# AegisIK/DistMLIP

Hardware: NVIDIA H100
Metric: atoms/sec (energy+forces) CHGNet a-Si r_cut=5A (higher is better)
Workload: dtype f32

## Files before the change

distmlip_b200/csrc/kernels.cu:

```cuda
#include "final_tail.cuh"
#include "kernels.cuh"
#include "wgmma.cuh"

#include <algorithm>

namespace b2m {

__device__ __forceinline__ float sigm(float x) {
  float e, r;
  asm("ex2.approx.ftz.f32 %0, %1;" : "=f"(e) : "f"(x * -1.4426950408889634f));
  asm("rcp.approx.ftz.f32 %0, %1;" : "=f"(r) : "f"(1.f + e));
  return r;
}
__device__ __forceinline__ float silu_f(float x) { return x * sigm(x); }
__device__ __forceinline__ float dsilu_f(float x) {
  float s = sigm(x);
  return s * (1.f + x * (1.f - s));
}

__device__ __forceinline__ uint32_t smem_u32(const void* p) { return (uint32_t)__cvta_generic_to_shared(p); }
__device__ __forceinline__ void mbar_init(uint64_t* bar, uint32_t count) {
  asm volatile("mbarrier.init.shared::cta.b64 [%0], %1;" ::"r"(smem_u32(bar)), "r"(count) : "memory");
}
__device__ __forceinline__ void fence_barrier_init() {
// ... 256 lines not shown
template <int ROWS>
__device__ __forceinline__ void issue_gather(const AtomConvArgs& a, int64_t t, const EdgeRow& row, int lr, float* buf,
                                             uint64_t* bar, int* s_src, int* s_dst, int* s_bond, float* s_d) {
  if (lr == 0) mbar_expect_tx(bar, (uint32_t)min((int64_t)ROWS, a.E - t * ROWS) * 512u);
  if (lr < ROWS) {
    if (s_src != nullptr) s_src[lr] = row.src;
    s_dst[lr] = row.dst;
    s_bond[lr] = row.bond;
    s_d[lr] = row.d;
    if (row.src >= 0) bulk_g2s(buf + lr * LDE, a.Aproj + (size_t)row.src * D2, 512u, bar);
  }
}
template <int ROWS>
__device__ __forceinline__ void radial_rows(const AtomConvArgs& a, const float* s_d, int nvalid, float* be_s, float* be8,
                                            float* dbe_s, float* dbe8) {
  const int r = threadIdx.x % ROWS, half = (threadIdx.x / ROWS) & 1;
  const float d = s_d[r];
  const int k0 = half ? 5 : 0, k1 = half ? 9 : 5;
  for (int k = k0; k < k1; k++) {
    float be = 0.f, dbe = 0.f;
    if (r < nvalid) rbf_env_k(d, a.rp.freq[k], a.rp, be, dbe);
    *(k < 8 ? be_s + r * 8 + k : be8 + r) = be;
    if (dbe_s != nullptr) *(k < 8 ? dbe_s + r * 8 + k : dbe8 + r) = dbe;
  }
}
__device__ __forceinline__ float2 ld_f2(const float* p) { return *reinterpret_cast<const float2*>(p); }
__device__ __forceinline__ void st_f2(float* p, float x, float y) { *reinterpret_cast<float2*>(p) = make_float2(x, y); }

__device__ __forceinline__ constexpr int fq(int ii, int j) { return 4 * (j >> 1) + 2 * ii + (j & 1); }

__device__ __forceinline__ void radial_mma(const Map& m, int h, const float* x_s, const float* img, float (&d)[32]) {
  const float2 u = ld_f2(x_s + m.row(2 * h) * 8 + m.cb), v = ld_f2(x_s + m.row(2 * h + 1) * 8 + m.cb);
  const float x[1][4] = {{u.x, v.x, u.y, v.y}};
  uint32_t b = s_u32(img);
  asm volatile("" : "+r"(b));
  wg_mma64(x, b, b + 512u * 4u, 0, false, d);
}

template <int R>
__device__ __forceinline__ void first_layer_half(const AtomConvArgs& a, const Map& m, int h, const float* tile,
                                                 const int* s_dst, const int* s_bond, const float* be_s,
                                                 const float* be8, const float* rad, int nvalid,
                                                 float (&acc)[R][AC]) {
  const int c0 = 64 * m.branch + m.cb;
  float2 cv[2][AC / 2], qv[2][AC / 2];
  float b8[2];
  bool viaQ[2], ok[2];
#pragma unroll
  for (int ii = 0; ii < 2; ii++) {
    const int r = m.row(2 * h + ii);
    const int dst = s_dst[r], bond = s_bond[r];
    ok[ii] = r < nvalid;
    viaQ[ii] = a.Qproj != nullptr && bond >= 0;
    const float* cp = a.Cproj + (size_t)max(dst, 0) * D2 + c0;
#pragma unroll
    for (int jj = 0; jj < AC / 2; jj++) cv[ii][jj] = dst >= 0 ? __ldg(reinterpret_cast<const float2*>(cp + 8 * jj)) : make_float2(0.f, 0.f);
    if (viaQ[ii]) {
      const float* qp = a.Qproj + (size_t)bond * D2 + c0;
#pragma unroll
      for (int jj = 0; jj < AC / 2; jj++) qv[ii][jj] = __ldg(reinterpret_cast<const float2*>(qp + 8 * jj));
    } else {
#pragma unroll
      for (int jj = 0; jj < AC / 2; jj++) qv[ii][jj] = make_float2(0.f, 0.f);
    }
    b8[ii] = be8[r];
  }
  float d[32];
  radial_mma(m, h, be_s, rad + ATOM_RAD_M + 1024 * m.branch, d);
#pragma unroll
  for (int j = 0; j < AC; j++) {
    const float m8 = rad[ATOM_RAD_M8 + 64 * m.branch + m.col(j)];
#pragma unroll
    for (int ii = 0; ii < 2; ii++) {
      const int r = m.row(2 * h + ii);
      const float x = tile[r * LDE + 64 * m.branch + m.col(j)];
      const float2 c2 = cv[ii][j >> 1], q2 = qv[ii][j >> 1];
      const float t = viaQ[ii] ? ((j & 1) ? q2.y : q2.x) : fmaf(b8[ii], m8, d[fq(ii, j)]);
      acc[2 * h + ii][j] = ok[ii] ? x + ((j & 1) ? c2.y : c2.x) + t : 0.f;
    }
  }
}

template <int R>
__device__ __forceinline__ void wg_mm64_acc(const float (&x)[R][AC], int h, const float* Bcan, float (&acc)[R][AC]) {
  float v[8][4];
#pragma unroll
  for (int ks = 0; ks < 8; ks++) {
    v[ks][0] = x[2 * h][2 * ks], v[ks][1] = x[2 * h + 1][2 * ks];
    v[ks][2] = x[2 * h][2 * ks + 1], v[ks][3] = x[2 * h + 1][2 * ks + 1];
  }
  const uint32_t b_hi = s_u32(Bcan);
  float d[32];
  wg_mma64(v, b_hi, b_hi + 4096u * 4u, 0, false, d);
#pragma unroll
  for (int q = 0; q < 32; q++) acc[2 * h + ((q >> 1) & 1)][2 * (q >> 2) + (q & 1)] = d[q];
}

__device__ __forceinline__ float quad_row_sum(const float (&v)[AR]) {
  const int l = threadIdx.x & 3;
  const bool b0 = l & 1, b1 = l & 2;
  float w[2];
#pragma unroll
  for (int h = 0; h < 2; h++)
    w[h] = (b0 ? v[2 * h + 1] : v[2 * h]) + __shfl_xor_sync(0xffffffffu, b0 ? v[2 * h] : v[2 * h + 1], 1);
  return (b1 ? w[1] : w[0]) + __shfl_xor_sync(0xffffffffu, b1 ? w[0] : w[1], 2);
}

__device__ __forceinline__ void red_add_v4(float* p, float4 v) {
  asm volatile("red.global.add.v4.f32 [%0], {%1, %2, %3, %4};" ::"l"(p), "f"(v.x), "f"(v.y), "f"(v.z), "f"(v.w)
               : "memory");
}

__device__ __forceinline__ void seg_add(float* out, int width, int col, int k, const float4& v, int& cur, float4& sum) {
  if (k != cur) {
    if (cur >= 0) red_add_v4(out + (size_t)cur * width + col, sum);
    cur = k;
    sum = make_float4(0.f, 0.f, 0.f, 0.f);
  }
  if (k >= 0) sum.x += v.x, sum.y += v.y, sum.z += v.z, sum.w += v.w;
}

template <int LPR, int ROWS = TM, int NTH = NT>
__device__ __forceinline__ void scatter_rows(const float* tile, const int* key0, float* out0, const int* key1,
                                             float* out1, const int* gidx, float* gat, const int* sidx = nullptr,
                                             float* sto = nullptr) {
  constexpr int R = ROWS * LPR / NTH, W = 4 * LPR, B = 8;
  static_assert(R % B == 0 && B % 4 == 0, "batches of B rows, their indices read as int4");
  const int t = threadIdx.x % NTH, q = t % LPR, r0 = t / LPR * R;
  float4 s0 = make_float4(0.f, 0.f, 0.f, 0.f), s1 = s0;
  int c0 = -1, c1 = -1;
#pragma unroll
  for (int b = 0; b < R; b += B) {
    float4 v[B];
    int k0[B], k1[B], kg[B], ks[B];
#pragma unroll
    for (int i = 0; i < B; i++) v[i] = *reinterpret_cast<const float4*>(tile + (r0 + b + i) * LDE + 4 * q);
    auto ld_idx = [&](const int* idx, bool on, int(&k)[B]) {
#pragma unroll
      for (int i = 0; i < B; i += 4) {
        const int4 x = on ? *reinterpret_cast<const int4*>(idx + r0 + b + i) : make_int4(-1, -1, -1, -1);
        k[i] = x.x, k[i + 1] = x.y, k[i + 2] = x.z, k[i + 3] = x.w;
      }
    };
    ld_idx(key0, out0 != nullptr, k0);
    ld_idx(key1, out1 != nullptr, k1);
    ld_idx(gidx, gat != nullptr, kg);
    ld_idx(sidx, sto != nullptr, ks);
#pragma unroll
    for (int i = 0; i < B; i++) {
      if (ks[i] >= 0) *reinterpret_cast<float4*>(sto + (size_t)ks[i] * W + 4 * q) = v[i];
      if (kg[i] >= 0) red_add_v4(gat + (size_t)kg[i] * W + 4 * q, v[i]);
      seg_add(out0, W, 4 * q, k0[i], v[i], c0, s0);
      seg_add(out1, W, 4 * q, k1[i], v[i], c1, s1);
    }
  }
  if (c0 >= 0) red_add_v4(out0 + (size_t)c0 * W + 4 * q, s0);
  if (c1 >= 0) red_add_v4(out1 + (size_t)c1 * W + 4 * q, s1);
}

constexpr int TW = 64;
constexpr int WGF = 3, NTF = 128 * WGF;
struct AtomSmemFwd {
  static constexpr int kTile = 32;
  static constexpr int kW = kTile + WGF * TW * LDE;
  static constexpr int kRad = kW + 16384;
  static constexpr int kBe = kRad + ATOM_RAD;
  static constexpr int kBe8 = kBe + WGF * TW * 8;
  static constexpr int kB2 = kBe8 + WGF * TW;
  static constexpr int kD = kB2 + 128;
  static constexpr int kIdx = kD + WGF * TW;
  static constexpr int kTotal = kIdx + 2 * WGF * TW;
  static constexpr size_t bytes = (size_t)kTotal * 4;
};
static_assert(AtomSmemFwd::bytes <= 232448, "atom-conv forward shared memory");
static_assert(AtomSmemFwd::kW % 4 == 0 && AtomSmemFwd::kRad % 4 == 0 && AtomSmemFwd::kBe % 4 == 0 &&
                  AtomSmemFwd::kIdx % 4 == 0,
              "16-byte aligned images, radial rows and index slots");

// ... 243 lines not shown
#pragma unroll
      for (int ii = 0; ii < 2; ii++)
#pragma unroll
        for (int jj = 0; jj < AC / 2; jj++) {
          float* p = P + m.row(ii) * LDE + c0 + m.col(2 * jj);
          const float2 pre = ld_f2(p);
          float& x0 = x[ii][2 * jj];
          float& x1 = x[ii][2 * jj + 1];
          x0 *= dsilu_f(pre.x);
          x1 *= dsilu_f(pre.y);
          st_f2(p, x0, x1);
        }
      float dm[32];
      radial_mma(m, 0, dbe_s, rad + ATOM_RAD_M + 1024 * mb.branch, dm);
#pragma unroll
      for (int ii = 0; ii < 2; ii++) {
        const int r = m.row(ii);
        const float db8 = dbe8[r];
        float s = 0.f;
#pragma unroll
        for (int jj = 0; jj < AC / 2; jj++) {
          const float2 mk = ld_f2(rad + ATOM_RAD_M8 + c0 + m.col(2 * jj));
          s = fmaf(x[ii][2 * jj], fmaf(db8, mk.x, dm[fq(ii, 2 * jj)]), s);
          s = fmaf(x[ii][2 * jj + 1], fmaf(db8, mk.y, dm[fq(ii, 2 * jj + 1)]), s);
        }
        if (r < nvalid && !(useQ && s_bond[r] >= 0)) sd[2 * mb.branch + ii] += s;
      }
    };
    reverse(mL, L);
    reverse(mG, G);
    {
      const float v = quad_row_sum(sd);
      const float v1 = __shfl_xor_sync(0xffffffffu, v, 2);
      const int r = m.row(tid & 1);
      if ((tid & 2) == 0 && r < nvalid) a.gd[e0 + r] += v + v1;
    }
    wg_sync(w);
    scatter_rows<32, TW, 128>(P, s_dst, a.gA != nullptr ? a.gC : nullptr, nullptr, nullptr, s_src, a.gA, s_bond,
                              useQ ? a.gQ : nullptr);
    fence_proxy_async_smem();
    wg_sync(w);
    if (t + step < ntiles) {
      issue_gather<TW>(a, t + step, nxt, lr, P, mbar, s_src, s_dst, s_bond, s_d);
      nxt = edge_row(a, (t + 2 * step) * TW + lr, lr < TW);
    }
  }
}

void launch_atomconv_bwd(cudaStream_t st, const AtomConvArgs& a, int num_sms) {
  if (a.E <= 0) return;
  static PerDeviceOnce attr;
  if (auto once_ = attr.first(); once_) {
    B2M_CK(cudaFuncSetAttribute(k_atomconv_bwd, cudaFuncAttributeMaxDynamicSharedMemorySize, (int)AtomSmemBwd::bytes));
  }
  launch(k_atomconv_bwd, std::min(cdiv(cdiv(a.E, TW), WGB), num_sms), NTB, AtomSmemBwd::bytes, st, a);
}

struct LineSmem {
  static constexpr int kBuf = 32;
  static constexpr int kW = kBuf + 2 * TM * LDE;
  static constexpr int kB2 = kW + 16384;
  static constexpr int kIdx = kB2 + 128;
  static constexpr int kTotal = kIdx + 6 * TM;
  static constexpr size_t bytes = (size_t)kTotal * 4;
};
static_assert(LineSmem::bytes <= 232448, "line-graph shared memory");

struct LineSm {
  float* smem;
  __device__ __forceinline__ uint64_t* hbar() const { return reinterpret_cast<uint64_t*>(smem); }
  __device__ __forceinline__ uint64_t* abar() const { return hbar() + 2; }
  __device__ __forceinline__ uint64_t* wbar() const { return hbar() + 4; }
  __device__ __forceinline__ float* buf(int s) const { return smem + LineSmem::kBuf + s * TM * LDE; }
  __device__ __forceinline__ float* W() const { return smem + LineSmem::kW; }
  __device__ __forceinline__ float* b2() const { return smem + LineSmem::kB2; }
  __device__ __forceinline__ int* idx(int s, int k) const {
    return reinterpret_cast<int*>(smem + LineSmem::kIdx) + (2 * k + s) * TM;
  }
};

struct AngleIdx {
  int a, b, c;
};
__device__ __forceinline__ AngleIdx angle_idx(const LineArgs& a, int64_t r) {
  AngleIdx x{-1, -1, -1};
  if (threadIdx.x < TM && r < a.A) {
    x.a = a.a_in[r];
    x.b = a.a_out[r];
    x.c = a.a_ctr[r];
  }
  return x;
}
__device__ __forceinline__ void line_issue_ha(const LineArgs& a, const LineSm& sm, int64_t t, const AngleIdx& x,
                                             float* buf, int s) {
  const int tid = threadIdx.x;
  if (tid == 0) mbar_expect_tx(&sm.hbar()[s], (uint32_t)min((int64_t)TM, a.A - t * TM) * 512u);
  if (tid < TM) {
    sm.idx(s, 0)[tid] = x.a;
    sm.idx(s, 1)[tid] = x.b;
    sm.idx(s, 2)[tid] = x.c;
    if (x.a >= 0) bulk_g2s(buf + tid * LDE, a.Ha + (size_t)x.a * D2, 512u, &sm.hbar()[s]);
  }
}
__device__ __forceinline__ void line_issue_ang(const LineArgs& a, const LineSm& sm, int64_t t, float* buf, int s) {
  const int tid = threadIdx.x;
  const int nvalid = (int)min((int64_t)TM, a.A - t * TM);
  if (tid == 0) mbar_expect_tx(&sm.abar()[s], (uint32_t)nvalid * 256u);
  if (tid < nvalid) bulk_g2s(buf + tid * LDE + 64, a.ang + (size_t)(t * TM + tid) * D, 256u, &sm.abar()[s]);
}
__device__ __forceinline__ AngleIdx line_prologue(const LineArgs& a, const LineSm& sm) {
  const int tid = threadIdx.x;
  if (tid == 0) {
    for (int i = 0; i < 5; i++) mbar_init(&sm.hbar()[i], 1);
    fence_barrier_init();
  }
  AngleIdx x = angle_idx(a, (int64_t)blockIdx.x * TM + tid);
  if (tid < 128) sm.b2()[tid] = a.b2 ? a.b2[tid] : 0.f;
  __syncthreads();
  if (tid == 0) bulk_g2s_image(sm.W(), a.Wgcan, 16384 * 4, sm.wbar());
  line_issue_ha(a, sm, blockIdx.x, x, sm.buf(0), 0);
  line_issue_ang(a, sm, blockIdx.x, sm.buf(1), 0);
  return angle_idx(a, ((int64_t)blockIdx.x + gridDim.x) * TM + tid);
}

__device__ __forceinline__ void line_first_layer(const LineArgs& a, const Map& m, const float* P, const int* s_b,
                                                 const int* s_c, int nvalid, float (&acc)[AR][AC]) {
  const int c0 = 64 * m.branch + m.cb;
#pragma unroll
  for (int i = 0; i < AR; i++) {
    const int r = m.row(i);
    const bool ok = r < nvalid;
    const float* hb = a.Hb + (size_t)(ok ? s_b[r] : 0) * D2 + c0;
    const float* xc = a.Xc + (size_t)(ok ? s_c[r] : 0) * D2 + c0;
    float2 hv[AC / 2], xv[AC / 2];
#pragma unroll
    for (int jj = 0; jj < AC / 2; jj++) {
      hv[jj] = ok ? __ldg(reinterpret_cast<const float2*>(hb + 8 * jj)) : make_float2(0.f, 0.f);
      xv[jj] = ok ? __ldg(reinterpret_cast<const float2*>(xc + 8 * jj)) : make_float2(0.f, 0.f);
    }
#pragma unroll
    for (int jj = 0; jj < AC / 2; jj++) {
      const float2 ha = ok ? ld_f2(P + r * LDE + c0 + 8 * jj) : make_float2(0.f, 0.f);
      float& x0 = acc[i][2 * jj];
      float& x1 = acc[i][2 * jj + 1];
      x0 = ok ? ha.x + x0 + hv[jj].x + xv[jj].x : 0.f;
      x1 = ok ? ha.y + x1 + hv[jj].y + xv[jj].y : 0.f;
    }
  }
}

__device__ __forceinline__ void red_add_v2(float* p, float x, float y) {
  asm volatile("red.global.add.v2.f32 [%0], {%1, %2};" ::"l"(p), "f"(x), "f"(y) : "memory");
}

template <bool HIDDEN>
__global__ void __launch_bounds__(NT, 1) k_line_fwd(const LineArgs a) {
  extern __shared__ __align__(128) float smem[];
  const LineSm sm{smem};
  const float* b2s = sm.b2();
  const int tid = threadIdx.x;
  const int64_t ntiles = (a.A + TM - 1) / TM, step = gridDim.x;
  AngleIdx nxt = line_prologue(a, sm);
  uint32_t wpar = 0;

  int it = 0;
  for (int64_t t = blockIdx.x; t < ntiles; t += step, it++) {
    const int s = it & 1;
    float* P = sm.buf(s);
    float* Q = sm.buf(s ^ 1);
    const int* s_b = sm.idx(s, 1);
    const int* s_c = sm.idx(s, 2);
    const int64_t r0 = t * TM;
    const int nvalid = (int)min((int64_t)TM, a.A - r0);
    const bool more = t + step < ntiles;
    const Map m;
    float acc[AR][AC];
    mbar_wait(&sm.abar()[s], stage_parity(it));
    mbar_wait(sm.wbar(), wpar);
    if (HIDDEN) wpar ^= 1;
    gemm64(Q, LDE, 64, sm.W() + m.branch * 8192, acc);
    fence_proxy_async_smem();
    __syncthreads();
    if (more) {
      line_issue_ha(a, sm, t + step, nxt, Q, s ^ 1);
      nxt = angle_idx(a, (t + 2 * step) * TM + tid);
    }
    if (HIDDEN && tid == 0) bulk_g2s_image(sm.W(), a.W2can, 16384 * 4, sm.wbar());
    mbar_wait(&sm.hbar()[s], stage_parity(it));
    line_first_layer(a, m, P, s_b, s_c, nvalid, acc);
#pragma unroll
    for (int i = 0; i < AR; i++)
#pragma unroll
      for (int j = 0; j < AC; j++) acc[i][j] = HIDDEN || m.branch == 0 ? silu_f(acc[i][j]) : sigm(acc[i][j]);
    if (HIDDEN) {
      mbar_wait(sm.wbar(), wpar);
      wpar ^= 1;
      wg_mm64_acc(acc, 0, sm.W() + m.branch * 8192, acc);
      wg_mm64_acc(acc, 1, sm.W() + m.branch * 8192, acc);
#pragma unroll
      for (int i = 0; i < AR; i++)
#pragma unroll
        for (int j = 0; j < AC; j++) {
          const float u = acc[i][j] + b2s[m.branch * 64 + m.col(j)];
          acc[i][j] = m.branch == 0 ? silu_f(u) : sigm(u);
        }
    }
    fence_proxy_async_smem();
    __syncthreads();
    if (more) {
      line_issue_ang(a, sm, t + step, P, s ^ 1);
      if (HIDDEN && tid == 0) bulk_g2s_image(sm.W(), a.Wgcan, 16384 * 4, sm.wbar());
    }
    if (m.branch == 1) {
#pragma unroll
      for (int i = 0; i < AR; i++)
#pragma unroll
        for (int jj = 0; jj < AC / 2; jj++) st_f2(P + m.row(i) * LDE + m.col(2 * jj), acc[i][2 * jj], acc[i][2 * jj + 1]);
    }
    __syncthreads();
    if (m.branch == 0) {
#pragma unroll
      for (int i = 0; i < AR; i++) {
        const int r = m.row(i);
        if (HIDDEN) {
#pragma unroll
          for (int jj = 0; jj < AC / 2; jj++) {
            float* p = P + r * LDE + m.col(2 * jj);
            const float2 g = ld_f2(p);
            st_f2(p, acc[i][2 * jj] * g.x, acc[i][2 * jj + 1] * g.y);
          }
        } else if (r < nvalid) {
          const float* ang = a.ang + (size_t)(r0 + r) * D;
          float* out = a.ang_out + (size_t)(r0 + r) * D;
          float2 av[AC / 2];
#pragma unroll
          for (int jj = 0; jj < AC / 2; jj++) av[jj] = __ldg(reinterpret_cast<const float2*>(ang + m.col(2 * jj)));
#pragma unroll
          for (int jj = 0; jj < AC / 2; jj++) {
            const int c = m.col(2 * jj);
            const float2 g = ld_f2(P + r * LDE + c);
            st_f2(out + c, av[jj].x + acc[i][2 * jj] * g.x, av[jj].y + acc[i][2 * jj + 1] * g.y);
          }
        }
      }
    }
    if (HIDDEN) {
      __syncthreads();
      scatter_rows<16>(P, s_b, a.aggB, nullptr, nullptr, nullptr, nullptr);
    }
  }
}

template <bool HIDDEN>
__global__ void __launch_bounds__(NT, 1) k_line_bwd(const LineArgs a) {
  extern __shared__ __align__(128) float smem[];
  const LineSm sm{smem};
  const float* b2s = sm.b2();
  const int tid = threadIdx.x;
  const int64_t ntiles = (a.A + TM - 1) / TM, step = gridDim.x;
  AngleIdx nxt = line_prologue(a, sm);
  uint32_t wpar = 0;

  int it = 0;
  for (int64_t t = blockIdx.x; t < ntiles; t += step, it++) {
    const int s = it & 1;
    float* P = sm.buf(s);
    float* H = sm.buf(s ^ 1);
    const int* s_a = sm.idx(s, 0);
    const int* s_b = sm.idx(s, 1);
    const int* s_c = sm.idx(s, 2);
    const int64_t r0 = t * TM;
    const int nvalid = (int)min((int64_t)TM, a.A - r0);
    const bool more = t + step < ntiles;
    const Map m;
    float acc[AR][AC];
    mbar_wait(&sm.abar()[s], stage_parity(it));
    mbar_wait(sm.wbar(), wpar);
    wpar ^= 1;
    gemm64(H, LDE, 64, sm.W() + m.branch * 8192, acc);
    __syncthreads();
    if (tid == 0) bulk_g2s_image(sm.W(), HIDDEN ? a.W2can : a.WgTcan, 16384 * 4, sm.wbar());
    mbar_wait(&sm.hbar()[s], stage_parity(it));
    line_first_layer(a, m, P, s_b, s_c, nvalid, acc);
    if (HIDDEN) {
#pragma unroll
      for (int i = 0; i < AR; i++)
#pragma unroll
        for (int jj = 0; jj < AC / 2; jj++) {
          float& x0 = acc[i][2 * jj];
          float& x1 = acc[i][2 * jj + 1];
          st_f2(P + m.row(i) * LDE + m.branch * 64 + m.col(2 * jj), x0, x1);
          x0 = silu_f(x0);
          x1 = silu_f(x1);
        }
      mbar_wait(sm.wbar(), wpar);
      wpar ^= 1;
    }
#pragma unroll
    for (int h = 0; h < 2; h++) {
      if (HIDDEN) wg_mm64_acc(acc, h, sm.W() + m.branch * 8192, acc);
#pragma unroll
      for (int ii = 0; ii < 2; ii++)
#pragma unroll
        for (int jj = 0; jj < AC / 2; jj++) {
          const int i = 2 * h + ii;
          const float u0 = HIDDEN ? acc[i][2 * jj] + b2s[m.branch * 64 + m.col(2 * jj)] : acc[i][2 * jj];
          const float u1 = HIDDEN ? acc[i][2 * jj + 1] + b2s[m.branch * 64 + m.col(2 * jj + 1)] : acc[i][2 * jj + 1];
          st_f2(H + m.row(i) * LDE + m.branch * 64 + m.col(2 * jj), m.branch == 0 ? u0 : sigm(u0),
                m.branch == 0 ? u1 : sigm(u1));
        }
    }
    __syncthreads();
    if (HIDDEN && tid == 0) bulk_g2s_image(sm.W(), a.W2Tcan, 16384 * 4, sm.wbar());
#pragma unroll
    for (int h = 0; h < 2; h++) {
      bool ok[2];
      float2 gm2[2][AC / 2];
#pragma unroll
      for (int ii = 0; ii < 2; ii++) {
        const int r = m.row(2 * h + ii);
        ok[ii] = r < nvalid;
        const float* gsrc =
            HIDDEN ? a.gaggB + (size_t)(ok[ii] ? s_b[r] : 0) * D : a.gang + (size_t)(r0 + (ok[ii] ? r : 0)) * D;
#pragma unroll
        for (int jj = 0; jj < AC / 2; jj++)
          gm2[ii][jj] = ok[ii] ? *reinterpret_cast<const float2*>(gsrc + m.col(2 * jj)) : make_float2(0.f, 0.f);
      }
#pragma unroll
      for (int ii = 0; ii < 2; ii++) {
        const int i = 2 * h + ii;
        const int r = m.row(i);
#pragma unroll
        for (int j = 0; j < AC; j++) {
          const float2 ow2 = ld_f2(H + r * LDE + m.branch * 64 + m.col(j & ~1));
          const float2 pt2 = ld_f2(H + r * LDE + (1 - m.branch) * 64 + m.col(j & ~1));
          const float x = (j & 1) ? ow2.y : ow2.x;
          const float pt = (j & 1) ? pt2.y : pt2.x;
          float g = 0.f;
          if (ok[ii]) {
            const float gm = (j & 1) ? gm2[ii][j >> 1].y : gm2[ii][j >> 1].x;
            if (m.branch == 0) {
              const float sg = sigm(x);
              g = gm * pt * (sg * (1.f + x * (1.f - sg)));
            } else {
              const float oL = silu_f(pt);
              g = gm * oL * x * (1.f - x);
            }
          }
          acc[i][j] = g;
        }
      }
      if (HIDDEN) {
        if (h == 0) mbar_wait(sm.wbar(), wpar);
        wg_mm64_acc(acc, h, sm.W() + m.branch * 8192, acc);
      }
#pragma unroll
      for (int ii = 0; ii < 2; ii++)
#pragma unroll
        for (int jj = 0; jj < AC / 2; jj++) {
          const int i = 2 * h + ii;
          float* p = P + m.row(i) * LDE + m.branch * 64 + m.col(2 * jj);
          if (HIDDEN) {
            const float2 pre = ld_f2(p);
            st_f2(p, acc[i][2 * jj] * dsilu_f(pre.x), acc[i][2 * jj + 1] * dsilu_f(pre.y));
          } else {
            st_f2(p, acc[i][2 * jj], acc[i][2 * jj + 1]);
          }
        }
    }
    if (HIDDEN) wpar ^= 1;
    fence_proxy_async_smem();
    __syncthreads();
    if (more) {
      line_issue_ha(a, sm, t + step, nxt, H, s ^ 1);
      nxt = angle_idx(a, (t + 2 * step) * TM + tid);
    }
    if (HIDDEN && tid == 0) bulk_g2s_image(sm.W(), a.WgTcan, 16384 * 4, sm.wbar());
    scatter_rows<32>(P, s_b, a.gHb, s_c, a.gXc, s_a, a.gHa);
    mbar_wait(sm.wbar(), wpar);
    wpar ^= 1;
    {
      float d[32];
      const uint32_t bh = s_u32(sm.W()), bl = bh + 64u * 128u * 4u;
      wg_mm64(P, LDE, 64 * m.branch, 0, bh, bl, 0, false, d);
      wg_mm64(P, LDE, 64 * m.branch, 64, bh, bl, 64, true, d);
#pragma unroll
      for (int q = 0; q < 32; q += 2) {
        const int r = 64 * m.branch + m.rb + 8 * ((q >> 1) & 1), c = 8 * (q >> 2) + m.cb;
        if (r < nvalid) red_add_v2(&a.gang[(size_t)(r0 + r) * D + c], d[q], d[q + 1]);
      }
    }
    fence_proxy_async_smem();
    __syncthreads();
    if (more) {
      line_issue_ang(a, sm, t + step, P, s ^ 1);
      if (tid == 0) bulk_g2s_image(sm.W(), a.Wgcan, 16384 * 4, sm.wbar());
    }
  }
}

void launch_line_fwd(cudaStream_t st, const LineArgs& a, bool hidden, int num_sms) {
  if (a.A <= 0) return;
  static PerDeviceOnce attr;
  if (auto once_ = attr.first(); once_) {
    B2M_CK(cudaFuncSetAttribute(k_line_fwd<true>, cudaFuncAttributeMaxDynamicSharedMemorySize, (int)LineSmem::bytes));
    B2M_CK(cudaFuncSetAttribute(k_line_fwd<false>, cudaFuncAttributeMaxDynamicSharedMemorySize, (int)LineSmem::bytes));
  }
  const int grid = std::min(cdiv(a.A, TM), num_sms);
  with_flags([&](auto kHidden) { launch(k_line_fwd<kHidden>, grid, NT, LineSmem::bytes, st, a); }, hidden);
}
void launch_line_bwd(cudaStream_t st, const LineArgs& a, bool hidden, int num_sms) {
  if (a.A <= 0) return;
  static PerDeviceOnce attr;
  if (auto once_ = attr.first(); once_) {
    B2M_CK(cudaFuncSetAttribute(k_line_bwd<true>, cudaFuncAttributeMaxDynamicSharedMemorySize, (int)LineSmem::bytes));
    B2M_CK(cudaFuncSetAttribute(k_line_bwd<false>, cudaFuncAttributeMaxDynamicSharedMemorySize, (int)LineSmem::bytes));
  }
  const int grid = std::min(cdiv(a.A, TM), num_sms);
  with_flags([&](auto kHidden) { launch(k_line_bwd<kHidden>, grid, NT, LineSmem::bytes, st, a); }, hidden);
}

constexpr int BNR = 128;
template <int MODE>
__global__ void __launch_bounds__(256) k_bond_node(int nb, const float4* __restrict__ b_vec, RadialParams rp,
                                                   const float* __restrict__ W ,
                                                   const float* __restrict__ x0 ,
                                                   const float* __restrict__ x1 , float* __restrict__ out,
                                                   float* __restrict__ gdb) {
  extern __shared__ float bn_smem[];
  float(*be_s)[12] = reinterpret_cast<float(*)[12]>(bn_smem);
  float(*dbe_s)[12] = reinterpret_cast<float(*)[12]>(bn_smem + BNR * 12);
  float* Ws = bn_smem + 2 * BNR * 12;
  float(*P)[68] = reinterpret_cast<float(*)[68]>(bn_smem + 2 * BNR * 12 + 576);
  const int b0 = blockIdx.x * BNR, tid = threadIdx.x;
  for (int i = tid; i < 576; i += 256) Ws[i] = W[i];
  for (int i = tid; i < BNR * 9; i += 256) {
    const int r = i / 9, k = i % 9;
    float be = 0.f, dbe = 0.f;
    if (b0 + r < nb) rbf_env_k(b_vec[b0 + r].w, rp.freq[k], rp, be, dbe);
    be_s[r][k] = be;
    dbe_s[r][k] = dbe;
  }
  __syncthreads();
  for (int i = tid; i < BNR * 16; i += 256) {
    const int r = i >> 4, c = (i & 15) * 4;
    float4 pv = make_float4(0.f, 0.f, 0.f, 0.f);
    if (b0 + r < nb) {
      const size_t o = (size_t)(b0 + r) * 64 + c;
      const float4 a0 = *reinterpret_cast<const float4*>(x0 + o);
      if (MODE == 2) {
        pv = a0;
      } else {
        float w[4] = {0.f, 0.f, 0.f, 0.f};
#pragma unroll
        for (int k = 0; k < 9; k++) {
          const float b = be_s[r][k];
#pragma unroll
          for (int j = 0; j < 4; j++) w[j] = fmaf(b, Ws[(c + j) * 9 + k], w[j]);
        }
        const float4 a1 = *reinterpret_cast<const float4*>(x1 + o);
        if (MODE == 0) {
          *reinterpret_cast<float4*>(out + o) = make_float4(a0.x + a1.x * w[0], a0.y + a1.y * w[1], a0.z + a1.z * w[2], a0.w + a1.w * w[3]);
        } else {
          *reinterpret_cast<float4*>(out + o) = make_float4(a0.x * w[0], a0.y * w[1], a0.z * w[2], a0.w * w[3]);
          pv = make_float4(a0.x * a1.x, a0.y * a1.y, a0.z * a1.z, a0.w * a1.w);
        }
      }
    }
    if (MODE != 0) *reinterpret_cast<float4*>(&P[r][c]) = pv;
  }
  if (MODE == 1 || MODE == 2) {
    __syncthreads();
    {
      const int r = tid >> 1, par = tid & 1;
      float tot = 0.f;
      for (int k = par; k < 9; k += 2) {
        float sacc = 0.f;
#pragma unroll 8
        for (int c = 0; c < 64; c++) sacc = fmaf(P[r][c], Ws[c * 9 + k], sacc);
        tot += sacc * dbe_s[r][k];
      }
      tot += __shfl_xor_sync(0xffffffffu, tot, 1);
      if (par == 0 && b0 + r < nb) gdb[b0 + r] += tot;
    }
  }
}
constexpr size_t kBondNodeSmem = (size_t)(2 * BNR * 12 + 576 + BNR * 68) * sizeof(float);
template <int MODE>
static void launch_bond_node(cudaStream_t st, int nb, const float4* b_vec, RadialParams rp, const float* W, const float* x0,
                             const float* x1, float* out, float* gdb) {
  static PerDeviceOnce attr;
  if (auto once_ = attr.first(); once_)
    B2M_CK(cudaFuncSetAttribute(k_bond_node<MODE>, cudaFuncAttributeMaxDynamicSharedMemorySize, (int)kBondNodeSmem));
  launch(k_bond_node<MODE>, cdiv(nb, BNR), 256, kBondNodeSmem, st, nb, b_vec, rp, W, x0, x1, out, gdb);
}
void launch_bond_update_fwd(cudaStream_t st, int nb, const float4* b_vec, RadialParams rp3, const float* W3bw,
                            const float* h, const float* upd, float* hout) {
  if (nb <= 0) return;
  launch_bond_node<0>(st, nb, b_vec, rp3, W3bw, h, upd, hout, nullptr);
}
void launch_bond_update_bwd(cudaStream_t st, int nb, const float4* b_vec, RadialParams rp3, const float* W3bw,
                            const float* gh, const float* upd, float* gupd, float* gdb) {
// ... 233 lines not shown
```

Before: 2.544 million.

## Split line-graph kernels into independent per-warpgroup tiles with register-sourced angle MMA

Restructures the line-graph forward and non-hidden backward kernels so each 128-thread warpgroup processes its own small tile of angles, with per-warpgroup mbarriers and index slots. CTA-wide double-buffered pipelines and __syncthreads are replaced by warpgroup-local sync. Weights are now staged once per CTA instead of being re-streamed every tile, and the angle features are loaded straight into registers as the wgmma A operand (3-term tf32 split), computing both the gate and core branches per warpgroup. The aim is to cut CTA-wide barrier stalls and repeated weight traffic. The cost is less cross-tile prefetch overlap and a changed shared-memory layout, and it relies on helpers like TW, stage_w and wg_sync defined elsewhere.

```diff
diff --git a/distmlip_b200/csrc/kernels.cu b/distmlip_b200/csrc/kernels.cu
--- a/distmlip_b200/csrc/kernels.cu
+++ b/distmlip_b200/csrc/kernels.cu
@@ -362,18 +362,27 @@
 }
 
 template <int R>
-__device__ __forceinline__ void wg_mm64_acc(const float (&x)[R][AC], int h, const float* Bcan, float (&acc)[R][AC]) {
-  float v[8][4];
+__device__ __forceinline__ void acc_frag(const float (&x)[R][AC], int h, float (&v)[8][4]) {
 #pragma unroll
   for (int ks = 0; ks < 8; ks++) {
     v[ks][0] = x[2 * h][2 * ks], v[ks][1] = x[2 * h + 1][2 * ks];
     v[ks][2] = x[2 * h][2 * ks + 1], v[ks][3] = x[2 * h + 1][2 * ks + 1];
   }
+}
+template <int R>
+__device__ __forceinline__ void frag_acc(const float (&d)[32], int h, float (&acc)[R][AC]) {
+#pragma unroll
+  for (int q = 0; q < 32; q++) acc[2 * h + ((q >> 1) & 1)][2 * (q >> 2) + (q & 1)] = d[q];
+}
+
+template <int R>
+__device__ __forceinline__ void wg_mm64_acc(const float (&x)[R][AC], int h, const float* Bcan, float (&acc)[R][AC]) {
+  float v[8][4];
+  acc_frag(x, h, v);
   const uint32_t b_hi = s_u32(Bcan);
   float d[32];
   wg_mma64(v, b_hi, b_hi + 4096u * 4u, 0, false, d);
-#pragma unroll
-  for (int q = 0; q < 32; q++) acc[2 * h + ((q >> 1) & 1)][2 * (q >> 2) + (q & 1)] = d[q];
+  frag_acc(d, h, acc);
 }
 
 __device__ __forceinline__ float quad_row_sum(const float (&v)[AR]) {
@@ -783,15 +792,16 @@
 struct AngleIdx {
   int a, b, c;
 };
-__device__ __forceinline__ AngleIdx angle_idx(const LineArgs& a, int64_t r) {
+__device__ __forceinline__ AngleIdx angle_row(const LineArgs& a, int64_t r, bool has_row) {
   AngleIdx x{-1, -1, -1};
-  if (threadIdx.x < TM && r < a.A) {
+  if (has_row && r < a.A) {
     x.a = a.a_in[r];
     x.b = a.a_out[r];
     x.c = a.a_ctr[r];
   }
   return x;
 }
+__device__ __forceinline__ AngleIdx angle_idx(const LineArgs& a, int64_t r) { return angle_row(a, r, threadIdx.x < TM); }
 __device__ __forceinline__ void line_issue_ha(const LineArgs& a, const LineSm& sm, int64_t t, const AngleIdx& x,
                                              float* buf, int s) {
   const int tid = threadIdx.x;
@@ -824,11 +834,12 @@
   return angle_idx(a, ((int64_t)blockIdx.x + gridDim.x) * TM + tid);
 }
 
+template <int R>
 __device__ __forceinline__ void line_first_layer(const LineArgs& a, const Map& m, const float* P, const int* s_b,
-                                                 const int* s_c, int nvalid, float (&acc)[AR][AC]) {
+                                                 const int* s_c, int nvalid, float (&acc)[R][AC]) {
   const int c0 = 64 * m.branch + m.cb;
 #pragma unroll
-  for (int i = 0; i < AR; i++) {
+  for (int i = 0; i < R; i++) {
     const int r = m.row(i);
     const bool ok = r < nvalid;
     const float* hb = a.Hb + (size_t)(ok ? s_b[r] : 0) * D2 + c0;
@@ -854,106 +865,192 @@
   asm volatile("red.global.add.v2.f32 [%0], {%1, %2};" ::"l"(p), "f"(x), "f"(y) : "memory");
 }
 
+template <int WG, int NIMG>
+struct LineSmemWg {
+  static constexpr int kBuf = 32;
+  static constexpr int kW = kBuf + WG * TW * LDE;
+  static constexpr int kB2 = kW + NIMG * 16384;
+  static constexpr int kIdx = kB2 + 128;
+  static constexpr int kTotal = kIdx + 3 * WG * TW;
+  static constexpr size_t bytes = (size_t)kTotal * 4;
+  static_assert(bytes <= 232448, "line-graph shared memory");
+  static_assert(kW % 32 == 0 && kIdx % 4 == 0, "128-byte aligned images, 16-byte aligned index slots");
+};
 template <bool HIDDEN>
-__global__ void __launch_bounds__(NT, 1) k_line_fwd(const LineArgs a) {
+struct LineFwd {
+  static constexpr int WG = HIDDEN ? 2 : 3;
+  using Smem = LineSmemWg<WG, HIDDEN ? 2 : 1>;
+};
+constexpr int LBWG = 2;
+using LineBwdSmem = LineSmemWg<LBWG, 2>;
+
+__device__ __forceinline__ void line_issue_ha_wg(const LineArgs& a, int64_t t, const AngleIdx& x, int lr, float* buf,
+                                                 uint64_t* bar, int* s_a, int* s_b, int* s_c) {
+  if (lr == 0) mbar_expect_tx(bar, (uint32_t)min((int64_t)TW, a.A - t * TW) * 512u);
+  if (lr < TW) {
+    s_a[lr] = x.a;
+    s_b[lr] = x.b;
+    s_c[lr] = x.c;
+    if (x.a >= 0) bulk_g2s(buf + lr * LDE, a.Ha + (size_t)x.a * D2, 512u, bar);
+  }
+}
+__device__ __forceinline__ void line_ang_frag(const LineArgs& a, const Map& m, int64_t r0, int nvalid, float (&x)[8][4]) {
+  float2 u[2][8];
+#pragma unroll
+  for (int ii = 0; ii < 2; ii++) {
+    const int r = m.row(ii);
+    const bool ok = r < nvalid;
+    const float* p = a.ang + (size_t)(r0 + (ok ? r : 0)) * D + m.cb;
+#pragma unroll
+    for (int ks = 0; ks < 8; ks++) u[ii][ks] = ok ? __ldg(reinterpret_cast<const float2*>(p + 8 * ks)) : make_float2(0.f, 0.f);
+  }
+#pragma unroll
+  for (int ks = 0; ks < 8; ks++) x[ks][0] = u[0][ks].x, x[ks][1] = u[1][ks].x, x[ks][2] = u[0][ks].y, x[ks][3] = u[1][ks].y;
+}
+__device__ __forceinline__ void wg_mma64_pair(const float (&x)[8][4], const float* Bcan, float (&L)[2][AC],
+                                              float (&G)[2][AC]) {
+  constexpr uint32_t LBO = 8 * 128;
+  uint32_t ah[8][4], al[8][4];
+#pragma unroll
+  for (int ks = 0; ks < 8; ks++)
+#pragma unroll
+    for (int q = 0; q < 4; q++) {
+      ah[ks][q] = tf32_hi_bits(x[ks][q]);
+      al[ks][q] = __float_as_uint(x[ks][q] - __uint_as_float(ah[ks][q]));
+    }
+  float dL[32], dG[32];
+  auto mma = [&](float(&d)[32], uint32_t b_hi) {
+#pragma unroll
+    for (int ks = 0; ks < 8; ks++)
+#pragma unroll
+      for (int term = 0; term < 3; term++) {
+        const uint64_t bd = gmma_desc((term == 2 ? b_hi + 4096u * 4u : b_hi) + ks * 2 * LBO, LBO, 128u);
+        wgmma_tf32_n64_rA(d, term == 1 ? al[ks] : ah[ks], bd, (ks > 0 || term > 0) ? 1 : 0);
+      }
+  };
+  const uint32_t b = s_u32(Bcan);
+  acc_fence(dL);
+  acc_fence(dG);
+  wgmma_fence();
+  mma(dL, b);
+  mma(dG, b + 8192u * 4u);
+  wgmma_commit();
+  wgmma_wait_all();
+  acc_fence(dL);
+  acc_fence(dG);
+  frag_acc(dL, 0, L);
+  frag_acc(dG, 0, G);
+}
+
+template <bool HIDDEN>
+__global__ void __launch_bounds__(128 * LineFwd<HIDDEN>::WG, 1) k_line_fwd(const LineArgs a) {
+  using S = typename LineFwd<HIDDEN>::Smem;
+  constexpr int WG = LineFwd<HIDDEN>::WG;
   extern __shared__ __align__(128) float smem[];
-  const LineSm sm{smem};
-  const float* b2s = sm.b2();
-  const int tid = threadIdx.x;
-  const int64_t ntiles = (a.A + TM - 1) / TM, step = gridDim.x;
-  AngleIdx nxt = line_prologue(a, sm);
-  uint32_t wpar = 0;
-
+  const int tid = threadIdx.x, w = tid >> 7, lr = tid & 127;
+  uint64_t* mbar = reinterpret_cast<uint64_t*>(smem) + w;
+  const float* Wg = smem + S::kW;
+  const float* W2 = smem + S::kW + 16384;
+  const float* b2s = smem + S::kB2;
+  float* P = smem + S::kBuf + w * TW * LDE;
+  int* s_a = reinterpret_cast<int*>(smem + S::kIdx) + w * TW;
+  int* s_b = reinterpret_cast<int*>(smem + S::kIdx) + (WG + w) * TW;
+  int* s_c = reinterpret_cast<int*>(smem + S::kIdx) + (2 * WG + w) * TW;
+
+  const int ntiles = (int)((a.A + TW - 1) / TW), first = WG * blockIdx.x + w, step = WG * gridDim.x;
+  if (tid == 0) {
+    for (int i = 0; i < WG; i++) mbar_init(reinterpret_cast<uint64_t*>(smem) + i, 1);
+    fence_barrier_init();
+  }
+  AngleIdx nxt = angle_row(a, (int64_t)first * TW + lr, lr < TW);
+  stage_w<128 * WG>(smem + S::kW, a.Wgcan, 4096);
+  if (HIDDEN) {
+    stage_w<128 * WG>(smem + S::kW + 16384, a.W2can, 4096);
+    if (tid < 128) smem[S::kB2 + tid] = a.b2[tid];
+  }
+  __syncthreads();
+  if (first < ntiles)
+    line_issue_ha_wg(a, first, nxt, lr, P, mbar, s_a, s_b, s_c);
+  nxt = angle_row(a, (int64_t)(first + step) * TW + lr, lr < TW);
+
+  const Map m;
+  Map mL = m, mG = m;
+  mL.branch = 0;
+  mG.branch = 1;
   int it = 0;
-  for (int64_t t = blockIdx.x; t < ntiles; t += step, it++) {
-    const int s = it & 1;
-    float* P = sm.buf(s);
-    float* Q = sm.buf(s ^ 1);
-    const int* s_b = sm.idx(s, 1);
-    const int* s_c = sm.idx(s, 2);
-    const int64_t r0 = t * TM;
-    const int nvalid = (int)min((int64_t)TM, a.A - r0);
-    const bool more = t + step < ntiles;
-    const Map m;
-    float acc[AR][AC];
-    mbar_wait(&sm.abar()[s], stage_parity(it));
-    mbar_wait(sm.wbar(), wpar);
-    if (HIDDEN) wpar ^= 1;
-    gemm64(Q, LDE, 64, sm.W() + m.branch * 8192, acc);
-    fence_proxy_async_smem();
-    __syncthreads();
-    if (more) {
-      line_issue_ha(a, sm, t + step, nxt, Q, s ^ 1);
-      nxt = angle_idx(a, (t + 2 * step) * TM + tid);
-    }
-    if (HIDDEN && tid == 0) bulk_g2s_image(sm.W(), a.W2can, 16384 * 4, sm.wbar());
-    mbar_wait(&sm.hbar()[s], stage_parity(it));
-    line_first_layer(a, m, P, s_b, s_c, nvalid, acc);
-#pragma unroll
-    for (int i = 0; i < AR; i++)
-#pragma unroll
-      for (int j = 0; j < AC; j++) acc[i][j] = HIDDEN || m.branch == 0 ? silu_f(acc[i][j]) : sigm(acc[i][j]);
-    if (HIDDEN) {
-      mbar_wait(sm.wbar(), wpar);
-      wpar ^= 1;
-      wg_mm64_acc(acc, 0, sm.W() + m.branch * 8192, acc);
-      wg_mm64_acc(acc, 1, sm.W() + m.branch * 8192, acc);
-#pragma unroll
-      for (int i = 0; i < AR; i++)
-#pragma unroll
-        for (int j = 0; j < AC; j++) {
-          const float u = acc[i][j] + b2s[m.branch * 64 + m.col(j)];
-          acc[i][j] = m.branch == 0 ? silu_f(u) : sigm(u);
+  for (int t = first; t < ntiles; t += step, it++) {
+    int64_t r0 = (int64_t)t * TW;
+    asm volatile("" : "+l"(r0));
+    const int nvalid = (int)min((int64_t)TW, a.A - r0);
+    float L[2][AC], G[2][AC];
+    {
+      float x[8][4];
+      line_ang_frag(a, m, r0, nvalid, x);
+      wg_sync(w);
+      wg_mma64_pair(x, Wg, L, G);
+    }
+    mbar_wait(mbar, (uint32_t)it & 1u);
+    line_first_layer(a, mL, P, s_b, s_c, nvalid, L);
+    line_first_layer(a, mG, P, s_b, s_c, nvalid, G);
+    if constexpr (!HIDDEN) {
+      fence_proxy_async_smem();
+      wg_sync(w);
+      if (t + step < ntiles) {
+        line_issue_ha_wg(a, t + step, nxt, lr, P, mbar, s_a, s_b, s_c);
+        nxt = angle_row(a, ((int64_t)t + 2 * step) * TW + lr, lr < TW);
+      }
+#pragma unroll
+      for (int ii = 0; ii < 2; ii++) {
+        const int r = m.row(ii);
+        if (r >= nvalid) continue;
+        const float* ang = a.ang + (size_t)(r0 + r) * D;
+        float* out = a.ang_out + (size_t)(r0 + r) * D;
+        float2 av[AC / 2];
+#pragma unroll
+        for (int jj = 0; jj < AC / 2; jj++) av[jj] = __ldg(reinterpret_cast<const float2*>(ang + m.col(2 * jj)));
+#pragma unroll
+        for (int jj = 0; jj < AC / 2; jj++) {
+          const float l0 = silu_f(L[ii][2 * jj]), l1 = silu_f(L[ii][2 * jj + 1]);
+          const float g0 = sigm(G[ii][2 * jj]), g1 = sigm(G[ii][2 * jj + 1]);
+          st_f2(out + m.col(2 * jj), av[jj].x + l0 * g0, av[jj].y + l1 * g1);
         }
-    }
-    fence_proxy_async_smem();
-    __syncthreads();
-    if (more) {
-      line_issue_ang(a, sm, t + step, P, s ^ 1);
-      if (HIDDEN && tid == 0) bulk_g2s_image(sm.W(), a.Wgcan, 16384 * 4, sm.wbar());
-    }
-    if (m.branch == 1) {
-#pragma unroll
-      for (int i = 0; i < AR; i++)
-#pragma unroll
-        for (int jj = 0; jj < AC / 2; jj++) st_f2(P + m.row(i) * LDE + m.col(2 * jj), acc[i][2 * jj], acc[i][2 * jj + 1]);
-    }
-    __syncthreads();
-    if (m.branch == 0) {
-#pragma unroll
-      for (int i = 0; i < AR; i++) {
-        const int r = m.row(i);
-        if (HIDDEN) {
-#pragma unroll
-          for (int jj = 0; jj < AC / 2; jj++) {
-            float* p = P + r * LDE + m.col(2 * jj);
-            const float2 g = ld_f2(p);
-            st_f2(p, acc[i][2 * jj] * g.x, acc[i][2 * jj + 1] * g.y);
-          }
-        } else if (r < nvalid) {
-          const float* ang = a.ang + (size_t)(r0 + r) * D;
-          float* out = a.ang_out + (size_t)(r0 + r) * D;
-          float2 av[AC / 2];
-#pragma unroll
-          for (int jj = 0; jj < AC / 2; jj++) av[jj] = __ldg(reinterpret_cast<const float2*>(ang + m.col(2 * jj)));
-#pragma unroll
-          for (int jj = 0; jj < AC / 2; jj++) {
-            const int c = m.col(2 * jj);
-            const float2 g = ld_f2(P + r * LDE + c);
-            st_f2(out + c, av[jj].x + acc[i][2 * jj] * g.x, av[jj].y + acc[i][2 * jj + 1] * g.y);
-          }
+      }
+    } else {
+#pragma unroll
+      for (int ii = 0; ii < 2; ii++)
+#pragma unroll
+        for (int j = 0; j < AC; j++) L[ii][j] = silu_f(L[ii][j]);
+      wg_mm64_acc(L, 0, W2, L);
+#pragma unroll
+      for (int ii = 0; ii < 2; ii++)
+#pragma unroll
+        for (int j = 0; j < AC; j++) L[ii][j] = silu_f(L[ii][j] + b2s[m.col(j)]);
+#pragma unroll
+      for (int ii = 0; ii < 2; ii++)
+#pragma unroll
+        for (int j = 0; j < AC; j++) G[ii][j] = silu_f(G[ii][j]);
+      wg_mm64_acc(G, 0, W2 + 8192, G);
+#pragma unroll
+      for (int ii = 0; ii < 2; ii++)
+#pragma unroll
+        for (int jj = 0; jj < AC / 2; jj++) {
+          const float g0 = sigm(G[ii][2 * jj] + b2s[64 + m.col(2 * jj)]);
+          const float g1 = sigm(G[ii][2 * jj + 1] + b2s[64 + m.col(2 * jj + 1)]);
+          st_f2(P + m.row(ii) * LDE + m.col(2 * jj), L[ii][2 * jj] * g0, L[ii][2 * jj + 1] * g1);
         }
-      }
-    }
-    if (HIDDEN) {
-      __syncthreads();
-      scatter_rows<16>(P, s_b, a.aggB, nullptr, nullptr, nullptr, nullptr);
-    }
-  }
-}
-
-template <bool HIDDEN>
-__global__ void __launch_bounds__(NT, 1) k_line_bwd(const LineArgs a) {
+      wg_sync(w);
+      scatter_rows<16, TW, 128>(P, s_b, a.aggB, nullptr, nullptr, nullptr, nullptr);
+      fence_proxy_async_smem();
+      wg_sync(w);
+      if (t + step < ntiles) {
+        line_issue_ha_wg(a, t + step, nxt, lr, P, mbar, s_a, s_b, s_c);
+        nxt = angle_row(a, ((int64_t)t + 2 * step) * TW + lr, lr < TW);
+      }
+    }
+  }
+}
+
+__device__ __forceinline__ void line_bwd_bond(const LineArgs& a) {
   extern __shared__ __align__(128) float smem[];
   const LineSm sm{smem};
   const float* b2s = sm.b2();
@@ -980,39 +1077,37 @@
     wpar ^= 1;
     gemm64(H, LDE, 64, sm.W() + m.branch * 8192, acc);
     __syncthreads();
-    if (tid == 0) bulk_g2s_image(sm.W(), HIDDEN ? a.W2can : a.WgTcan, 16384 * 4, sm.wbar());
+    if (tid == 0) bulk_g2s_image(sm.W(), a.W2can, 16384 * 4, sm.wbar());
     mbar_wait(&sm.hbar()[s], stage_parity(it));
     line_first_layer(a, m, P, s_b, s_c, nvalid, acc);
-    if (HIDDEN) {
-#pragma unroll
-      for (int i = 0; i < AR; i++)
-#pragma unroll
-        for (int jj = 0; jj < AC / 2; jj++) {
-          float& x0 = acc[i][2 * jj];
-          float& x1 = acc[i][2 * jj + 1];
-          st_f2(P + m.row(i) * LDE + m.branch * 64 + m.col(2 * jj), x0, x1);
-          x0 = silu_f(x0);
-          x1 = silu_f(x1);
-        }
-      mbar_wait(sm.wbar(), wpar);
-      wpar ^= 1;
-    }
+#pragma unroll
+    for (int i = 0; i < AR; i++)
+#pragma unroll
+      for (int jj = 0; jj < AC / 2; jj++) {
+        float& x0 = acc[i][2 * jj];
+        float& x1 = acc[i][2 * jj + 1];
+        st_f2(P + m.row(i) * LDE + m.branch * 64 + m.col(2 * jj), x0, x1);
+        x0 = silu_f(x0);
+        x1 = silu_f(x1);
+      }
+    mbar_wait(sm.wbar(), wpar);
+    wpar ^= 1;
 #pragma unroll
     for (int h = 0; h < 2; h++) {
-      if (HIDDEN) wg_mm64_acc(acc, h, sm.W() + m.branch * 8192, acc);
+      wg_mm64_acc(acc, h, sm.W() + m.branch * 8192, acc);
 #pragma unroll
       for (int ii = 0; ii < 2; ii++)
 #pragma unroll
         for (int jj = 0; jj < AC / 2; jj++) {
           const int i = 2 * h + ii;
-          const float u0 = HIDDEN ? acc[i][2 * jj] + b2s[m.branch * 64 + m.col(2 * jj)] : acc[i][2 * jj];
-          const float u1 = HIDDEN ? acc[i][2 * jj + 1] + b2s[m.branch * 64 + m.col(2 * jj + 1)] : acc[i][2 * jj + 1];
+          const float u0 = acc[i][2 * jj] + b2s[m.branch * 64 + m.col(2 * jj)];
+          const float u1 = acc[i][2 * jj + 1] + b2s[m.branch * 64 + m.col(2 * jj + 1)];
           st_f2(H + m.row(i) * LDE + m.branch * 64 + m.col(2 * jj), m.branch == 0 ? u0 : sigm(u0),
                 m.branch == 0 ? u1 : sigm(u1));
         }
     }
     __syncthreads();
-    if (HIDDEN && tid == 0) bulk_g2s_image(sm.W(), a.W2Tcan, 16384 * 4, sm.wbar());
+    if (tid == 0) bulk_g2s_image(sm.W(), a.W2Tcan, 16384 * 4, sm.wbar());
 #pragma unroll
     for (int h = 0; h < 2; h++) {
       bool ok[2];
@@ -1021,8 +1116,7 @@
       for (int ii = 0; ii < 2; ii++) {
         const int r = m.row(2 * h + ii);
         ok[ii] = r < nvalid;
-        const float* gsrc =
-            HIDDEN ? a.gaggB + (size_t)(ok[ii] ? s_b[r] : 0) * D : a.gang + (size_t)(r0 + (ok[ii] ? r : 0)) * D;
+        const float* gsrc = a.gaggB + (size_t)(ok[ii] ? s_b[r] : 0) * D;
 #pragma unroll
         for (int jj = 0; jj < AC / 2; jj++)
           gm2[ii][jj] = ok[ii] ? *reinterpret_cast<const float2*>(gsrc + m.col(2 * jj)) : make_float2(0.f, 0.f);
@@ -1051,32 +1145,26 @@
           acc[i][j] = g;
         }
       }
-      if (HIDDEN) {
-        if (h == 0) mbar_wait(sm.wbar(), wpar);
-        wg_mm64_acc(acc, h, sm.W() + m.branch * 8192, acc);
-      }
+      if (h == 0) mbar_wait(sm.wbar(), wpar);
+      wg_mm64_acc(acc, h, sm.W() + m.branch * 8192, acc);
 #pragma unroll
       for (int ii = 0; ii < 2; ii++)
 #pragma unroll
         for (int jj = 0; jj < AC / 2; jj++) {
           const int i = 2 * h + ii;
           float* p = P + m.row(i) * LDE + m.branch * 64 + m.col(2 * jj);
-          if (HIDDEN) {
-            const float2 pre = ld_f2(p);
-            st_f2(p, acc[i][2 * jj] * dsilu_f(pre.x), acc[i][2 * jj + 1] * dsilu_f(pre.y));
-          } else {
-            st_f2(p, acc[i][2 * jj], acc[i][2 * jj + 1]);
-          }
+          const float2 pre = ld_f2(p);
+          st_f2(p, acc[i][2 * jj] * dsilu_f(pre.x), acc[i][2 * jj + 1] * dsilu_f(pre.y));
         }
     }
-    if (HIDDEN) wpar ^= 1;
+    wpar ^= 1;
     fence_proxy_async_smem();
     __syncthreads();
     if (more) {
       line_issue_ha(a, sm, t + step, nxt, H, s ^ 1);
       nxt = angle_idx(a, (t + 2 * step) * TM + tid);
     }
-    if (HIDDEN && tid == 0) bulk_g2s_image(sm.W(), a.WgTcan, 16384 * 4, sm.wbar());
+    if (tid == 0) bulk_g2s_image(sm.W(), a.WgTcan, 16384 * 4, sm.wbar());
     scatter_rows<32>(P, s_b, a.gHb, s_c, a.gXc, s_a, a.gHa);
     mbar_wait(sm.wbar(), wpar);
     wpar ^= 1;
@@ -1100,25 +1188,143 @@
   }
 }
 
+__device__ __forceinline__ void line_bwd_angle(const LineArgs& a) {
+  using S = LineBwdSmem;
+  constexpr int WG = LBWG;
+  extern __shared__ __align__(128) float smem[];
+  const int tid = threadIdx.x, w = tid >> 7, lr = tid & 127;
+  uint64_t* mbar = reinterpret_cast<uint64_t*>(smem) + w;
+  const float* Wg = smem + S::kW;
+  const float* WgT = smem + S::kW + 16384;
+  float* P = smem + S::kBuf + w * TW * LDE;
+  int* s_a = reinterpret_cast<int*>(smem + S::kIdx) + w * TW;
+  int* s_b = reinterpret_cast<int*>(smem + S::kIdx) + (WG + w) * TW;
+  int* s_c = reinterpret_cast<int*>(smem + S::kIdx) + (2 * WG + w) * TW;
+
+  const int ntiles = (int)((a.A + TW - 1) / TW), first = WG * blockIdx.x + w, step = WG * gridDim.x;
+  if (tid == 0) {
+    for (int i = 0; i < WG; i++) mbar_init(reinterpret_cast<uint64_t*>(smem) + i, 1);
+    fence_barrier_init();
+  }
+  AngleIdx nxt = angle_row(a, (int64_t)first * TW + lr, lr < TW);
+  stage_w<128 * WG>(smem + S::kW, a.Wgcan, 4096);
+  stage_w<128 * WG>(smem + S::kW + 16384, a.WgTcan, 4096);
+  __syncthreads();
+  if (first < ntiles)
+    line_issue_ha_wg(a, first, nxt, lr, P, mbar, s_a, s_b, s_c);
+  nxt = angle_row(a, (int64_t)(first + step) * TW + lr, lr < TW);
+
+  const Map m;
+  Map mL = m, mG = m;
+  mL.branch = 0;
+  mG.branch = 1;
+  int it = 0;
+  for (int t = first; t < ntiles; t += step, it++) {
+    int64_t r0 = (int64_t)t * TW;
+    asm volatile("" : "+l"(r0));
+    const int nvalid = (int)min((int64_t)TW, a.A - r0);
+    bool ok[2];
+    float2 gm2[2][AC / 2];
+#pragma unroll
+    for (int ii = 0; ii < 2; ii++) {
+      const int r = m.row(ii);
+      ok[ii] = r < nvalid;
+      const float* gsrc = a.gang + (size_t)(r0 + (ok[ii] ? r : 0)) * D;
+#pragma unroll
+      for (int jj = 0; jj < AC / 2; jj++)
+        gm2[ii][jj] = ok[ii] ? *reinterpret_cast<const float2*>(gsrc + m.col(2 * jj)) : make_float2(0.f, 0.f);
+    }
+    float L[2][AC], G[2][AC];
+    {
+      float x[8][4];
+      line_ang_frag(a, m, r0, nvalid, x);
+      wg_sync(w);
+      wg_mma64_pair(x, Wg, L, G);
+    }
+    mbar_wait(mbar, (uint32_t)it & 1u);
+    line_first_layer(a, mL, P, s_b, s_c, nvalid, L);
+    line_first_layer(a, mG, P, s_b, s_c, nvalid, G);
+#pragma unroll
+    for (int ii = 0; ii < 2; ii++) {
+#pragma unroll
+      for (int j = 0; j < AC; j++) {
+        const float u = L[ii][j], oG = sigm(G[ii][j]);
+        float gu = 0.f, gv = 0.f;
+        if (ok[ii]) {
+          const float gm = (j & 1) ? gm2[ii][j >> 1].y : gm2[ii][j >> 1].x;
+          const float sg = sigm(u);
+          gu = gm * oG * (sg * (1.f + u * (1.f - sg)));
+          gv = gm * silu_f(u) * oG * (1.f - oG);
+        }
+        L[ii][j] = gu;
+        G[ii][j] = gv;
+      }
+#pragma unroll
+      for (int jj = 0; jj < AC / 2; jj++) {
+        st_f2(P + m.row(ii) * LDE + m.col(2 * jj), L[ii][2 * jj], L[ii][2 * jj + 1]);
+        st_f2(P + m.row(ii) * LDE + 64 + m.col(2 * jj), G[ii][2 * jj], G[ii][2 * jj + 1]);
+      }
+    }
+    wg_sync(w);
+    scatter_rows<32, TW, 128>(P, s_b, a.gHb, s_c, a.gXc, s_a, a.gHa);
+    fence_proxy_async_smem();
+    wg_sync(w);
+    if (t + step < ntiles) {
+      line_issue_ha_wg(a, t + step, nxt, lr, P, mbar, s_a, s_b, s_c);
+      nxt = angle_row(a, ((int64_t)t + 2 * step) * TW + lr, lr < TW);
+    }
+    {
+      float v[8][4], d[32];
+      const uint32_t bh = s_u32(WgT), bl = bh + 64u * 128u * 4u;
+      acc_frag(L, 0, v);
+      wg_mma64(v, bh, bl, 0, false, d);
+      acc_frag(G, 0, v);
+      wg_mma64(v, bh, bl, 64, true, d);
+#pragma unroll
+      for (int q = 0; q < 32; q += 2) {
+        const int r = m.rb + 8 * ((q >> 1) & 1), c = 8 * (q >> 2) + m.cb;
+        if (r < nvalid) red_add_v2(&a.gang[(size_t)(r0 + r) * D + c], d[q], d[q + 1]);
+      }
+    }
+  }
+}
+
+static_assert(128 * LBWG == NT, "both backward kernels run 256-thread CTAs");
+template <bool HIDDEN>
+__global__ void __launch_bounds__(NT, 1) k_line_bwd(const LineArgs a) {
+  if constexpr (HIDDEN)
+    line_bwd_bond(a);
+  else
+    line_bwd_angle(a);
+}
+
 void launch_line_fwd(cudaStream_t st, const LineArgs& a, bool hidden, int num_sms) {
   if (a.A <= 0) return;
   static PerDeviceOnce attr;
   if (auto once_ = attr.first(); once_) {
-    B2M_CK(cudaFuncSetAttribute(k_line_fwd<true>, cudaFuncAttributeMaxDynamicSharedMemorySize, (int)LineSmem::bytes));
-    B2M_CK(cudaFuncSetAttribute(k_line_fwd<false>, cudaFuncAttributeMaxDynamicSharedMemorySize, (int)LineSmem::bytes));
-  }
-  const int grid = std::min(cdiv(a.A, TM), num_sms);
-  with_flags([&](auto kHidden) { launch(k_line_fwd<kHidden>, grid, NT, LineSmem::bytes, st, a); }, hidden);
+    B2M_CK(cudaFuncSetAttribute(k_line_fwd<true>, cudaFuncAttributeMaxDynamicSharedMemorySize,
+                                (int)LineFwd<true>::Smem::bytes));
+    B2M_CK(cudaFuncSetAttribute(k_line_fwd<false>, cudaFuncAttributeMaxDynamicSharedMemorySize,
+                                (int)LineFwd<false>::Smem::bytes));
+  }
+  with_flags(
+      [&](auto kHidden) {
+        using F = LineFwd<decltype(kHidden)::value>;
+        launch(k_line_fwd<kHidden>, std::min(cdiv(cdiv(a.A, TW), F::WG), num_sms), 128 * F::WG, F::Smem::bytes, st, a);
+      },
+      hidden);
 }
 void launch_line_bwd(cudaStream_t st, const LineArgs& a, bool hidden, int num_sms) {
   if (a.A <= 0) return;
   static PerDeviceOnce attr;
   if (auto once_ = attr.first(); once_) {
     B2M_CK(cudaFuncSetAttribute(k_line_bwd<true>, cudaFuncAttributeMaxDynamicSharedMemorySize, (int)LineSmem::bytes));
-    B2M_CK(cudaFuncSetAttribute(k_line_bwd<false>, cudaFuncAttributeMaxDynamicSharedMemorySize, (int)LineSmem::bytes));
-  }
-  const int grid = std::min(cdiv(a.A, TM), num_sms);
-  with_flags([&](auto kHidden) { launch(k_line_bwd<kHidden>, grid, NT, LineSmem::bytes, st, a); }, hidden);
+    B2M_CK(cudaFuncSetAttribute(k_line_bwd<false>, cudaFuncAttributeMaxDynamicSharedMemorySize, (int)LineBwdSmem::bytes));
+  }
+  if (hidden)
+    launch(k_line_bwd<true>, std::min(cdiv(a.A, TM), num_sms), NT, LineSmem::bytes, st, a);
+  else
+    launch(k_line_bwd<false>, std::min(cdiv(cdiv(a.A, TW), LBWG), num_sms), NT, LineBwdSmem::bytes, st, a);
 }
 
 constexpr int BNR = 128;
```

Result: faster. 2.640 million, median of 6 (+3.7%).
